# Priberam/Enhance-CB-Whisper

Hardware: AMD Instinct MI355X
Metric: utterances/sec (30 s clips) + keywords/sec matched, Whisper-large-v3 LEF 10k kw (higher is better)
Workload: dtype bf16

## Files before the change

### enhance-cb-whisper_amd/cbw/_lib.py

```python
from __future__ import annotations

import ctypes
import os

import torch

_HERE = os.path.dirname(os.path.abspath(__file__))
LIB_PATH = os.environ.get("CBW_LIB", os.path.join(_HERE, "libcbw.so"))

c_int, c_int64, c_float, c_void_p, c_char_p = ctypes.c_int, ctypes.c_int64, ctypes.c_float, ctypes.c_void_p, ctypes.c_char_p


class KwsConfig(ctypes.Structure):
    _fields_ = [("n_layers", c_int), ("embedding_dim", c_int), ("variant", c_int), ("proj_units", c_int),
                ("resnet_depth", c_int)]


class EncoderConfig(ctypes.Structure):
    _fields_ = [("n_mel", c_int), ("d_model", c_int), ("n_layers", c_int), ("n_heads", c_int), ("ffn_dim", c_int)]


class DecoderConfig(ctypes.Structure):
    _fields_ = [("vocab", c_int), ("d_model", c_int), ("n_layers", c_int), ("n_heads", c_int), ("ffn_dim", c_int),
                ("max_len", c_int)]
# ... 17 lines not shown
    "cbw_kws_rescore": (c_int, [c_void_p, c_void_p, c_void_p, c_void_p, c_void_p, c_int, c_int, c_int, c_void_p, c_int,
                                c_void_p, c_void_p, c_int64, c_void_p]),
    "cbw_kws_calibrate_bias": (c_int, [c_void_p, c_void_p, c_void_p, c_void_p, c_void_p, c_int, c_int, c_int, c_void_p,
                                       c_int, c_void_p, c_int64, c_void_p]),
    "cbw_kws_rescore_x3_workspace_bytes": (c_int64, [c_void_p, c_int, c_int]),
    "cbw_kws_rescore_x3": (c_int, [c_void_p, c_void_p, c_void_p, c_void_p, c_void_p, c_int, c_int, c_int, c_void_p,
                                   c_int, c_void_p, c_void_p, c_int64, c_void_p]),
    "cbw_kws_workspace_bytes": (c_int64, [c_void_p, c_int, c_int, c_int]),
    "cbw_kws_score": (c_int, [c_void_p, c_void_p, c_void_p, c_void_p, c_void_p, c_int, c_int, c_int, c_void_p,
                              c_void_p, c_int, c_void_p, c_int64, c_void_p]),
    "cbw_kws_classify": (c_int, [c_void_p, c_void_p, c_int, c_int, c_int, c_void_p, c_int, c_void_p, c_int64,
                                 c_void_p]),
    "cbw_kws_spot": (c_int, [c_void_p, c_void_p, c_int, c_float, c_int, c_void_p, c_void_p, c_void_p, c_void_p]),
    "cbw_checksum_workspace_bytes": (ctypes.c_int64, []),
    "cbw_checksum": (c_int, [c_void_p, ctypes.c_int64, c_void_p, c_void_p, ctypes.c_int64, c_void_p]),
    "cbw_kws_band": (c_int, [c_void_p, c_void_p, c_int, c_float, c_float, c_void_p, c_void_p, c_void_p]),
    "cbw_beam_select": (c_int, [c_void_p, c_void_p, c_int, c_int, c_int, c_void_p, c_void_p, c_void_p, c_void_p,
                                c_void_p, c_void_p, c_void_p, c_void_p, c_void_p, c_int, c_int, c_void_p]),
    "cbw_kws_set_score_offset": (c_int, [c_void_p, c_void_p]),
    "cbw_kws_band_scaled": (c_int, [c_void_p, c_void_p, c_int, c_float, c_float, c_void_p, c_void_p, c_void_p]),
    "cbw_kws_score_resized_workspace_bytes": (c_int64, [c_void_p, c_void_p, c_int, c_int, c_int, c_int, c_int, c_int]),
    "cbw_kws_score_resized": (c_int, [c_void_p, c_void_p, c_int, c_void_p, c_int, c_int, c_void_p, c_void_p, c_int,
                                      c_int, c_int, c_void_p, c_int, c_void_p, c_int64, c_void_p]),
    "cbw_mel": (c_int, [c_void_p, c_int64, c_int, c_void_p, c_void_p, c_int, c_void_p, c_void_p]),
    "cbw_mel_long": (c_int, [c_void_p, c_int64, c_int, c_void_p, c_void_p, c_void_p]),
    "cbw_encoder_create": (c_int, [ctypes.POINTER(EncoderConfig), ctypes.POINTER(c_void_p)]),
    "cbw_encoder_destroy": (c_int, [c_void_p]),
    "cbw_encoder_set_param": (c_int, [c_void_p, c_char_p, c_void_p, c_int64]),
    "cbw_encoder_finalize": (c_int, [c_void_p]),
    "cbw_encoder_workspace_bytes": (c_int64, [c_void_p, c_int]),
    "cbw_encoder_hs": (c_int, [c_void_p, c_void_p, c_int, c_void_p, c_int, c_int, c_void_p, c_void_p, c_int64,
                               c_void_p]),
    "cbw_conv2d": (c_int, [c_void_p, c_void_p, c_void_p, c_void_p, c_void_p] + [c_int] * 12 + [c_void_p]),
    "cbw_conv1x1_dual": (c_int, [c_void_p] * 6 + [c_int] * 10 + [c_void_p]),
    "cbw_gemm_splitk_factor": (c_int, [c_int, c_int, c_int]),
    "cbw_gemm": (c_int, [c_void_p] * 5 + [c_int] * 5 + [c_void_p, c_int64, c_void_p]),
    "cbw_encoder_attention": (c_int, [c_void_p, c_void_p, c_int, c_int, c_int, c_void_p]),
    "cbw_kws_profile": (c_int, [c_void_p, c_int]),
    "cbw_decoder_create": (c_int, [ctypes.POINTER(DecoderConfig), ctypes.POINTER(c_void_p)]),
    "cbw_decoder_destroy": (c_int, [c_void_p]),
    "cbw_decoder_set_param": (c_int, [c_void_p, c_char_p, c_void_p, c_int64]),
    "cbw_decoder_finalize": (c_int, [c_void_p]),
    "cbw_decoder_vocab_padded": (c_int, [c_void_p]),
    "cbw_decoder_state_bytes": (c_int64, [c_void_p, c_int, c_int]),
    "cbw_decoder_cross_kv": (c_int, [c_void_p, c_void_p, c_int, c_void_p, c_int64, c_int, c_void_p]),
    "cbw_decoder_step": (c_int, [c_void_p, c_void_p, c_int, c_int, c_int, c_void_p, c_int64, c_void_p, c_void_p]),
    "cbw_decoder_step_dev": (c_int, [c_void_p, c_void_p, c_void_p, c_int, c_int, c_void_p, c_int64, c_void_p, c_void_p]),
    "cbw_decoder_prefill": (c_int, [c_void_p, c_void_p, c_int, c_int, c_int, c_void_p, c_int64, c_void_p, c_void_p]),
    "cbw_decoder_cross_kv_slot": (c_int, [c_void_p, c_void_p, c_int, c_int, c_void_p, c_int64, c_int, c_void_p]),
    "cbw_decoder_prefill_rows": (c_int, [c_void_p, c_void_p, c_int, c_int, c_int, c_int, c_int, c_int, c_void_p, c_int64,
                                         c_void_p, c_void_p]),
    "cbw_decoder_step_rows": (c_int, [c_void_p, c_void_p, c_void_p, c_int, c_int, c_void_p, c_int64, c_void_p, c_void_p]),
    "cbw_decoder_reorder": (c_int, [c_void_p, c_void_p, c_int, c_int, c_int, c_void_p, c_int64, c_void_p]),
    "cbw_decoder_cross_attn_probs": (c_int, [c_void_p, c_void_p, c_int, c_void_p, c_int, c_int, c_int, c_void_p,
                                             c_int64, c_void_p, c_void_p]),
    "cbw_dtw": (c_int, [c_void_p, c_int, c_int, c_void_p, c_void_p, c_void_p]),
    "cbw_logprob_topk": (c_int, [c_void_p, c_int, c_int, c_int, c_void_p, c_int64, c_int, c_void_p, c_void_p, c_void_p]),
    "cbw_timestamp_rules": (c_int, [c_void_p, c_int, c_int, c_int, c_void_p, c_void_p, c_int, c_int, c_int, c_int,
                                    c_void_p, c_void_p]),
    "cbw_kws_profile_read": (c_int, [c_void_p, ctypes.POINTER(ctypes.c_double), ctypes.POINTER(ctypes.c_double), ctypes.POINTER(c_int)]),
    "cbw_kws_profile_records": (c_int, [c_void_p, c_void_p, c_void_p, c_void_p, c_int]),
    "cbw_kws_profile_tiers": (c_int, [c_void_p, c_void_p, c_int]),
    "cbw_kws_profile_kernels": (c_int, [c_void_p, c_void_p, c_int]),
    "cbw_kws_calibrate_fp8": (c_int, [c_void_p, c_void_p, c_void_p, c_void_p, c_void_p, c_int, c_int, c_int, c_void_p,
                                      c_int, c_float, c_void_p, c_int64, c_void_p]),
    "cbw_kws_score_fp8": (c_int, [c_void_p, c_void_p, c_void_p, c_void_p, c_void_p, c_int, c_int, c_int, c_void_p,
# ... 63 lines not shown
```

### enhance-cb-whisper_amd/csrc/cbw_kernels.h

```cpp
#pragma once
#include <hip/hip_runtime.h>
#include <stdint.h>

#include <initializer_list>
#include <string>

typedef __bf16 bf16;

enum {
    CBW_EPI_RELU = 1,
    CBW_EPI_GELU = 2,
    CBW_EPI_RES_F32 = 4,
    CBW_EPI_OUT_F32 = 8,
    CBW_EPI_RES_AFTER_ACT = 16,
    CBW_EPI_SPLIT3 = 32,
    CBW_EPI_RES_SPLIT = 64
};

struct ConvArgs {
    const void* x;
    const void* w;
    const float* bias;
    const void* res;
    void* y;
// ... 49 lines not shown
int cbw_gemv_waves(int K);
bool cbw_gemv_ln_ok(int M, int K);
hipError_t cbw_gemv(const GemvArgs& a, hipStream_t st);

struct F8ConvArgs {
    const uint8_t* x;
    const uint8_t* w;
    const float* alpha;
    const float* bias;
    const uint8_t* res;
    float res_scale;
    void* y;
    float y_inv_scale;
    int out_bf16;
    const void* zero;
    int N, H, W, Cin, Ho, Wo, Cout, KH, KW, sh, sw, ph, pw, M;
    int relu;
};
bool cbw_conv_fp8_supported(const F8ConvArgs& a);
bool cbw_conv_fp8_stream_supported(const F8ConvArgs& a);
hipError_t cbw_conv_fp8_stream(const F8ConvArgs& a, hipStream_t st);
hipError_t cbw_conv_fp8(const F8ConvArgs& a, hipStream_t st);
hipError_t cbw_quant_fp8(const uint16_t* x, uint8_t* y, int64_t n, float inv_scale, hipStream_t st);
int cbw_absmax_groups();
hipError_t cbw_absmax_f32(const float* x, int64_t n, float* part, hipStream_t st);
hipError_t cbw_mfma_fp8_probe(const uint8_t* A, const uint8_t* Bt, float* C, int mode, hipStream_t st);
hipError_t cbw_cvt_fp8_probe(const float* x, uint8_t* q, float* back, int n, hipStream_t st);

bool cbw_conv_ring_supported(const ConvArgs& a);
hipError_t cbw_conv_ring(const ConvArgs& a, hipStream_t st);
bool cbw_conv_stream_supported(const ConvArgs& a);
bool cbw_conv_stream_wanted(const ConvArgs& a);
hipError_t cbw_conv_stream(const ConvArgs& a, hipStream_t st);

hipError_t cbw_bottleneck_s1(const uint16_t* x, uint16_t* y, const uint16_t* wr, const float* br, const uint16_t* wm,
                             const float* bm, const uint16_t* we, const float* be, const void* zero, int N, int H,
                             int W, hipStream_t st);
hipError_t cbw_bottleneck_s1_q8(const uint16_t* x, uint8_t* y, const uint16_t* wr, const float* br, const uint16_t* wm,
                                const float* bm, const uint16_t* we, const float* be, float inv_scale, int N, int H,
                                int W, hipStream_t st);
hipError_t cbw_bottleneck_s1_first(const uint16_t* x, uint16_t* y, const uint16_t* wr, const float* br,
                                   const uint16_t* wm, const float* bm, const uint16_t* wcat, const float* bcat,
                                   const void* zero, int N, int H, int W, hipStream_t st);

hipError_t cbw_cast_permute_lbtd(const float* x, uint16_t* y, int B, int L, int T, int D, hipStream_t st);
hipError_t cbw_normalize_rows(const void* x, int x_is_f32, void* y, int y_is_f32, int L, int B, int T, int E,
                              float eps, int permute_lb, hipStream_t st);
hipError_t cbw_nchw_to_nhwc4(const float* x, uint16_t* y, int K, int L, int H, int W, hipStream_t st);
hipError_t cbw_l2norm_rows_f32(float* x, int64_t rows, int E, hipStream_t st);
hipError_t cbw_lef_time_project(const float* x, const float* w, const float* b, void* y, int y_is_f32,
                                const float* mask_in, float* mask_out,
                                int L, int B, int T, int U, float eps, hipStream_t st);
hipError_t cbw_sim_maps(const uint16_t* kwd, const float* kwd_mask, const uint16_t* utt, const float* utt_mask,
                        uint16_t* out, int K, int L, int Tk, int Tu, int E, hipStream_t st);
hipError_t cbw_sim_to_nchw(const uint16_t* maps, float* out, int K, int L, int Tk, int Tu, hipStream_t st);
hipError_t cbw_stem_conv(const uint16_t* x, const uint16_t* w, const float* bias, uint16_t* y,
                         int N, int H, int W, int Ho, int Wo, hipStream_t st);
hipError_t cbw_stem_pool(const uint16_t* x, const uint16_t* w, const float* bias, uint16_t* y, int N, int H, int W,
                         int Hs, int Ws, int Hp, int Wp, hipStream_t st);
hipError_t cbw_stem16_pool(const uint16_t* x, const uint16_t* w, const float* bias, uint16_t* y, int N, int H,
                           int W, int Hs, int Ws, int Hp, int Wp, hipStream_t st);
hipError_t cbw_stem16_pool_x3(const uint16_t* x, const uint16_t* w, const float* bias, uint16_t* y, int N, int H,
                              int W, int Hs, int Ws, int Hp, int Wp, hipStream_t st);
hipError_t cbw_maps_split16(const float* x, uint16_t* y, int K, int L, int H, int W, hipStream_t st);
hipError_t cbw_sim_resize(const float* sim, int64_t layer_stride, int ld, const int* off_dev, int k0, int K, int L,
                          int Tu, int Ho, int Wo, uint16_t* out, hipStream_t st);
// ... 68 lines not shown
```

### enhance-cb-whisper_amd/csrc/conv_stream.hip

```cpp
#include "cbw_common.h"
#include "cbw_kernels.h"

typedef int cs_i32x4 __attribute__((ext_vector_type(4)));
__device__ cs_i32x4 cs_raw_load(cs_i32x4 rsrc, int voffset, int soffset, int aux)
    __asm("llvm.amdgcn.raw.buffer.load.v4i32");
__device__ void cs_raw_store(cs_i32x4 vdata, cs_i32x4 rsrc, int voffset, int soffset, int aux)
    __asm("llvm.amdgcn.raw.buffer.store.v4i32");

namespace {

constexpr int CS_NSTEP = 64;
constexpr int CS_WBYTES = 131072;
constexpr int CS_MAXSLICE = 1024;

CBW_DEV cs_i32x4 cs_rsrc(const void* base, uint32_t bytes) {
    const uint64_t p = (uint64_t)base;
    cs_i32x4 r{(int)(uint32_t)p, (int)(uint32_t)(p >> 32), (int)bytes, 0x00020000};
#pragma unroll
    for (int q = 0; q < 4; ++q) r[q] = __builtin_amdgcn_readfirstlane(r[q]);
    return r;
}
CBW_DEV cs_i32x4 cs_load(cs_i32x4 rsrc, int voff, int soff) { return cs_raw_load(rsrc, voff, soff, 0); }
CBW_DEV void cs_store(cs_i32x4 v, cs_i32x4 rsrc, int voff, int soff) { cs_raw_store(v, rsrc, voff, soff, 0); }

// ... 116 lines not shown
            }
#pragma unroll
            for (int h = 0; h < 2; ++h) {
                const int nl = s * CS_NSTEP + h * 32 + fq * 8;
                const f32x4 bv0 = *(const f32x4*)(bias_s + nl), bv1 = *(const f32x4*)(bias_s + nl + 4);
#pragma unroll
                for (int pf = 0; pf < PF; ++pf) {
                    float v[8];
#pragma unroll
                    for (int q = 0; q < 4; ++q) {
                        v[q] = acc[pf][2 * h][q] + bv0[q];
                        v[4 + q] = acc[pf][2 * h + 1][q] + bv1[q];
                    }
                    if (has_res) {
                        const bf16x8 rv = __builtin_bit_cast(bf16x8, rs[pf][h]);
#pragma unroll
                        for (int q = 0; q < 8; ++q) v[q] += bf2f(rv[q]);
                    }
                    bf16x8 o;
#pragma unroll
                    for (int q = 0; q < 8; ++q) o[q] = f2bf(relu ? fmaxf(v[q], 0.f) : v[q]);
                    const int yo = (exp & 2) ? (v[0] == 12345.f ? yoff[pf] : OOR) : yoff[pf];
                    cs_store(__builtin_bit_cast(cs_i32x4, o), yr, yo, (n_lo + s * CS_NSTEP + h * 32) * 2);
                }
            }
            if (has_res && s + RD < nsteps) load_res(rs, s + RD);
        };
        for (int s = 0; s < nsteps; s += RD) {
            if (PN && s + RD >= nsteps && u + ustride < units) load_rows(u + ustride, xn, roffn, yoffn);
#pragma unroll
            for (int r = 0; r < RD; ++r) step(res[r], s + r);
        }
    }
}

int num_cus_cs() {
    static int n = 0;
    if (n == 0) {
        int dev = 0;
        (void)hipGetDevice(&dev);
        if (hipDeviceGetAttribute(&n, hipDeviceAttributeMultiprocessorCount, dev) != hipSuccess || n <= 0) n = 256;
        const char* e = getenv("CBW_CS_CUS");
        if (e && atoi(e) > 0) n = std::min(n, atoi(e));
    }
    return n;
}

int cs_exp() {
    const char* e = getenv("CBW_CS_EXP");
    return e ? atoi(e) : 0;
}

int stream_prefetch() {
    const char* e = getenv("CBW_CS_PREFETCH");
    return e ? atoi(e) : -1;
}

int stream_k512() {
    const char* e = getenv("CBW_CS_K512");
    return e ? atoi(e) : 1;
}

int stream_mode() {
    const char* e = getenv("CBW_CONV_STREAM");
    return e ? atoi(e) : 1;
}
// ... 35 lines not shown
    const int ktot = a.Cin + (a.x2 ? a.Cin2 : 0);
    const int sn = slice_channels(a.Cout, ktot);
    const int nslice = a.Cout / sn;
    const int cus = cbw_cs_grid_cus > 0 ? std::min(num_cus_cs(), cbw_cs_grid_cus) : num_cus_cs();
    const int G = 8 * nslice * std::max(1, cus / (8 * nslice));
    const size_t lds = (size_t)sn * ktot * 2 + (size_t)sn * 4;
    const int pf = stream_prefetch();
    const int pn = pf >= 0 ? pf : (ktot == 128 || (ktot == 256 && !a.res));
#define CS_LAUNCH(KS, WAVES, RD, PFD, PN)                                                                               \
    do {                                                                                                           \
        cbw_last_conv_kernel = "conv_stream_kernel<" #KS ", " #WAVES ", " #RD ", " #PFD ", " #PN ">";                \
        hipLaunchKernelGGL((conv_stream_kernel<KS, WAVES, RD, PFD, PN>), dim3(G), dim3(WAVES * 64), lds, st, a,       \
                           nslice, sn, cs_exp());                                                                  \
    } while (0)
    switch (ktot) {
        case 128:
            if (pn) CS_LAUNCH(4, 8, 2, 2, 1);
            else CS_LAUNCH(4, 12, 2, 2, 0);
            break;
        case 256:
            if (pn) CS_LAUNCH(8, 8, 1, 2, 1);
            else CS_LAUNCH(8, 12, 1, 2, 0);
            break;
        case 512:
            CS_LAUNCH(16, 8, 2, 1, 0);
            break;
        default:
            CS_LAUNCH(12, 8, 2, 2, 0);
            break;
    }
#undef CS_LAUNCH
    return hipGetLastError();
}
```

### enhance-cb-whisper_amd/csrc/runtime.cpp

```cpp
#include <hip/hip_runtime.h>

#include <algorithm>
#include <cmath>
#include <cstring>
#include <limits>
#include <map>
#include <memory>
#include <string>
#include <vector>

#include "cbw.h"
#include "cbw_kernels.h"

namespace {

thread_local std::string g_err;

int fail(int code, const std::string& msg) {
    g_err = msg;
    return code;
}

#define HIPCHK(expr)                                                                                   \
    do {                                                                                               \
// ... 153 lines not shown
    int cin, H, W, stride;
};

int launch_conv(const ConvW& c, const void* x, int N, int H, int W, void* y, const void* res, int flags,
                const void* zero, hipStream_t st, int* Ho_out = nullptr, int* Wo_out = nullptr, Prof* prof = nullptr,
                const Src2* src2 = nullptr, float* splitk_ws = nullptr) {
    ConvArgs a{};
    a.x = x; a.w = c.w.p; a.bias = c.b.as<float>(); a.res = res; a.y = y; a.zero = zero;
    if (src2) { a.x2 = src2->x; a.Cin2 = src2->cin; a.H2 = src2->H; a.W2 = src2->W; a.s2 = src2->stride; }
    a.N = N; a.H = H; a.W = W; a.Cin = c.cin; a.Cout = c.cout; a.KH = c.k; a.KW = c.k;
    a.sh = a.sw = c.stride; a.ph = a.pw = c.k / 2;
    a.Ho = (H + 2 * a.ph - a.KH) / a.sh + 1;
    a.Wo = (W + 2 * a.pw - a.KW) / a.sw + 1;
    a.M = N * a.Ho * a.Wo;
    a.res_ld = a.y_ld = c.cout;
    a.flags = flags | (c.relu ? CBW_EPI_RELU : 0);
    if (Ho_out) *Ho_out = a.Ho;
    if (Wo_out) *Wo_out = a.Wo;
    const bool rec = prof && prof->on && (size_t)(2 * prof->used + 1) < prof->ev.size();
    if (rec) HIPCHK(hipEventRecord(prof->ev[2 * prof->used], st));
    cbw_last_conv_kernel = "?";
    if (splitk_ws) HIPCHK(cbw_conv_igemm_splitk(a, cbw_conv_splitk_factor(a), splitk_ws, st));
    else HIPCHK(cbw_conv_igemm(a, st));
    if (rec) {
        HIPCHK(hipEventRecord(prof->ev[2 * prof->used + 1], st));
        prof->flop[prof->used] = 2.0 * a.M * a.Cout * ((double)a.Cin * a.KH * a.KW + (a.x2 ? a.Cin2 : 0));
        prof->tier[prof->used] = prof->cur_tier;
        prof->kern[prof->used] = cbw_last_conv_kernel;
        prof->used++;
    }
    return CBW_OK;
}

size_t align_up(size_t n) { return (n + 255) & ~(size_t)255; }

struct BlockW {
    ConvW conv[3];
    int nconv = 0;
    bool has_sc = false;
    bool fused_sc = false;
    ConvW sc;
    std::string prefix;
    int stage = 0;
};

struct ConvF8 {
    DevBuf w, alpha, b;
    int cin = 0, cout = 0, k = 1, stride = 1;
    bool relu = false;
};
struct BlockF8 {
    ConvF8 conv[3];
    bool has_sc = false;
    ConvF8 sc;
    float s_x = 1.f, s_t1 = 1.f, s_t2 = 1.f, s_sc = 1.f;
    float s_out = 1.f;
    bool out_bf16 = false;
};

struct ConvW32 {
    DevBuf w, b;
    int cin = 0, cout = 0, k = 1, stride = 1;
    bool relu = false;
};
struct BlockW32 {
    ConvW32 conv[3];
    int nconv = 0;
    bool has_sc = false;
    ConvW32 sc;
};

int load_conv_bn32(const ParamStore& ps, const std::string& prefix, ConvW32& c) {
    std::vector<float> o, sh;
    CHK(fold_conv_host(ps, prefix, c.cin, c.cout, c.k, o, sh));
// ... 194 lines not shown
                        o[((co * 7 + kh) * 8 + kw) * C + c] = (*w)[((co * L + c) * 7 + kh) * 7 + kw] * sc[co];
        CHK(h->stem_w.upload(to_bf16(o)));
        CHK(h->stem_b.upload(sh));
    }
    h->blocks.clear();
    int cin = 64;
    for (size_t s = 0; s < hs.size(); ++s) {
        const int cout = hs[s];
        for (int li = 0; li < depths[s]; ++li) {
            const int stride = (li == 0 && s > 0) ? 2 : 1;
            const std::string p = root + ".encoder.stages." + std::to_string(s) + ".layers." + std::to_string(li);
            BlockW b;
            b.prefix = p;
            b.stage = (int)s + 1;
            if (cin != cout || stride != 1) {
                b.has_sc = true;
                b.sc.cin = cin; b.sc.cout = cout; b.sc.k = 1; b.sc.stride = stride; b.sc.relu = false;
                CHK(load_conv_bn(h->ps, p + ".shortcut", b.sc));
            }
            if (bottleneck) {
                const int mid = cout / 4;
                const int ci[3] = {cin, mid, mid}, co[3] = {mid, mid, cout}, k[3] = {1, 3, 1}, st[3] = {1, stride, 1};
                const bool rl[3] = {true, true, false};
                b.nconv = 3;
                for (int j = 0; j < 3; ++j) {
                    b.conv[j].cin = ci[j]; b.conv[j].cout = co[j]; b.conv[j].k = k[j]; b.conv[j].stride = st[j];
                    b.conv[j].relu = rl[j];
                    if (j == 2 && b.has_sc && cout % 128 == 0 && sc_fusion_enabled()) {
                        CHK(load_fused_expand_shortcut(h->ps, p + ".layer.2", p + ".shortcut", mid, cin, cout, b.conv[2]));
                        b.fused_sc = true;
                    } else {
                        CHK(load_conv_bn(h->ps, p + ".layer." + std::to_string(j), b.conv[j]));
                    }
                }
            } else {
                b.nconv = 2;
                b.conv[0].cin = cin; b.conv[0].cout = cout; b.conv[0].k = 3; b.conv[0].stride = stride; b.conv[0].relu = true;
                b.conv[1].cin = cout; b.conv[1].cout = cout; b.conv[1].k = 3; b.conv[1].stride = 1; b.conv[1].relu = false;
                for (int j = 0; j < 2; ++j) CHK(load_conv_bn(h->ps, p + ".layer." + std::to_string(j), b.conv[j]));
            }
            h->blocks.push_back(std::move(b));
            cin = cout;
        }
    }
    int rc;
    const auto* fw = h->ps.get("model.classifier.1.weight", (size_t)2 * h->hidden, &rc);
    if (!fw) return rc;
    const auto* fb = h->ps.get("model.classifier.1.bias", 2, &rc);
    if (!fb) return rc;
    CHK(h->fc_w.upload(*fw));
    CHK(h->fc_b.upload(*fb));
    CHK(h->fc_b16.upload(*fb));
    CHK(h->fc_b8.upload(*fb));
    return CBW_OK;
}

int build_projector(cbw_kws* h) {
    const int L = h->cfg.n_layers, D = h->cfg.embedding_dim, U = h->cfg.proj_units;
    h->p1.clear();
    h->p2.clear();
    h->p1.resize(L);
    h->p2.resize(L);
    for (int l = 0; l < L; ++l) {
        int rc;
        const std::string p = "projector." + std::to_string(l);
        const auto* w1 = h->ps.get(p + ".0.weight", (size_t)(D / 2) * D, &rc); if (!w1) return rc;
// ... 318 lines not shown
                        nullptr, 0, h->zero.p, st));
        CHK(launch_conv(h->p2[l], h1 + (size_t)l * rows_l * (D / 2), 1, 1, (int)rows_l, h2 + (size_t)l * rows_l * U,
                        nullptr, CBW_EPI_OUT_F32, h->zero.p, st));
    }
    if (h->cfg.variant == 1) {
        HIPCHK(cbw_normalize_rows(h2, 1, out, 0, L, B, T, U, eps, 1, st));
        HIPCHK(hipMemcpyAsync(mask_out, mask, sizeof(float) * B * L * T, hipMemcpyDeviceToDevice, st));
    } else {
        HIPCHK(cbw_lef_time_project(h2, h->tp_w.as<float>(), h->tp_b.as<float>(), out, 0, mask, mask_out, L, B, T, U, eps,
                                    st));
    }
    return CBW_OK;
}

}

namespace {
int64_t chunk_ws_bytes(const cbw_kws* h, int Tk, int Tu, int chunk) {
    const KwsPlan p = kws_plan(h, Tk, Tu, chunk);
    return (int64_t)(align_up(p.maps * 2) + 3 * align_up(p.big * 2) + 2 * align_up(p.small * 2));
}
}

extern "C" {

int64_t cbw_kws_workspace_bytes(cbw_kws* h, int Tk, int Tu, int chunk) {
    if (!h || !h->finalized || chunk <= 0) return -1;
    return kws_streams() * chunk_ws_bytes(h, Tk, Tu, chunk);
}

namespace {
int cs_shared_cus() {
    const char* e = getenv("CBW_CS_SHARED_CUS");
    return e ? atoi(e) : 96;
}
struct ChunkStreams {
    cbw_kws* h;
    hipStream_t st;
    int n;
    int saved_cus;
    static int balanced(int want, int nchunks) {
        const int n = std::max(1, std::min(want, nchunks));
        const int rounds = (nchunks + n - 1) / n;
        return std::max(1, (nchunks + rounds - 1) / rounds);
    }
    ChunkStreams(cbw_kws* h_, hipStream_t st_, int nchunks)
        : h(h_), st(st_), n(h_->fork_ev ? balanced(kws_streams(), nchunks) : 1), saved_cus(cbw_cs_grid_cus) {
        if (n > 1) cbw_cs_grid_cus = cs_shared_cus();
    }
    ~ChunkStreams() { cbw_cs_grid_cus = saved_cus; }
    ChunkStreams(const ChunkStreams&) = delete;
    ChunkStreams& operator=(const ChunkStreams&) = delete;
    int begin() {
        if (n > 1) {
            HIPCHK(hipEventRecord(h->fork_ev, st));
            for (int i = 0; i + 1 < n; ++i) {
                if (!h->side[i]) HIPCHK(side_stream_create(&h->side[i]));
                HIPCHK(hipStreamWaitEvent(h->side[i], h->fork_ev, 0));
            }
        }
        return CBW_OK;
    }
    hipStream_t stream(int i) const { return (i % n) ? h->side[i % n - 1] : st; }
    int slot(int i) const { return i % n; }
    int end() {
        for (int i = 0; i + 1 < n; ++i) {
            HIPCHK(hipEventRecord(h->join_ev[i], h->side[i]));
// ... 5 lines not shown

int resnet_chunk(cbw_kws* h, const KwsPlan& plan, char* ws, int kc, int Tk, int Tu, float* logits, hipStream_t st,
                 bool fp8 = false) {
    char* p = ws + align_up(plan.maps * 2);
    uint16_t* maps = (uint16_t*)ws;
    uint16_t* X = (uint16_t*)p; p += align_up(plan.big * 2);
    uint16_t* Y = (uint16_t*)p; p += align_up(plan.big * 2);
    uint16_t* SC = (uint16_t*)p; p += align_up(plan.big * 2);
    uint16_t* T1 = (uint16_t*)p; p += align_up(plan.small * 2);
    uint16_t* T2 = (uint16_t*)p;
    const int Hs = (Tk + 6 - 7) / 2 + 1, Ws = (Tu + 6 - 7) / 2 + 1;
    const int Hp = (Hs - 1) / 2 + 1, Wp = (Ws - 1) / 2 + 1;
    const int L = h->cfg.n_layers;

    auto stem = [&](int n0, int nn) -> int {
        uint16_t* xo = X + (size_t)n0 * Hp * Wp * 64;
        const uint16_t* mo = maps + (size_t)n0 * Tk * Tu * stem_channels(L);
        if (stem_channels(L) == 16) {
            HIPCHK(cbw_stem16_pool(mo, h->stem_w.as<uint16_t>(), h->stem_b.as<float>(), xo, nn, Tk, Tu, Hs, Ws, Hp, Wp,
                                   st));
        } else if (stem_fusion_enabled()) {
            HIPCHK(cbw_stem_pool(mo, h->stem_w.as<uint16_t>(), h->stem_b.as<float>(), xo, nn, Tk, Tu, Hs, Ws, Hp, Wp,
                                 st));
        } else {
            uint16_t* yo = Y + (size_t)n0 * Hs * Ws * 64;
            HIPCHK(cbw_stem_conv(mo, h->stem_w.as<uint16_t>(), h->stem_b.as<float>(), yo, nn, Tk, Tu, Hs, Ws, st));
            HIPCHK(cbw_maxpool3s2(yo, xo, nn, Hs, Ws, 64, Hp, Wp, st));
        }
        return CBW_OK;
    };
    auto blocks = [&](size_t b0, size_t b1, int n0, int nn, uint16_t*& x, uint16_t*& y, int& H, int& W,
                      int& C) -> int {
        auto at = [&](uint16_t* base, int hh, int ww, int cc) { return base + (size_t)n0 * hh * ww * cc; };
        for (size_t bi = b0; bi < b1; ++bi) {
            const auto& b = h->blocks[bi];
            uint16_t* xo = at(x, H, W, C);
            int Ho = H, Wo = W;
            const void* res = xo;
            const bool s1_first = b.nconv == 3 && b.has_sc && b.fused_sc && b.sc.stride == 1 && b.sc.cin == 64 &&
                                  b.conv[0].cin == 64 && b.conv[0].cout == 64 && b.conv[1].stride == 1 &&
                                  b.conv[2].cout == 256 && bottleneck_fusion_enabled() && bottleneck_first_enabled();
            if (b.has_sc && !b.fused_sc) {
                const int hs = (H - 1) / b.sc.stride + 1, ws2 = (W - 1) / b.sc.stride + 1;
                uint16_t* sco = at(SC, hs, ws2, b.sc.cout);
                CHK(launch_conv(b.sc, xo, nn, H, W, sco, nullptr, 0, h->zero.p, st, nullptr, nullptr, &h->prof));
                res = sco;
            }
            if (s1_first || (b.nconv == 3 && !b.has_sc && b.conv[0].cin == 256 && b.conv[0].cout == 64 &&
                             b.conv[2].cout == 256 && bottleneck_fusion_enabled())) {
                uint16_t* yo = at(y, H, W, 256);
                const bool rec = h->prof.on && (size_t)(2 * h->prof.used + 1) < h->prof.ev.size();
                if (rec) HIPCHK(hipEventRecord(h->prof.ev[2 * h->prof.used], st));
                if (s1_first)
                    HIPCHK(cbw_bottleneck_s1_first(xo, yo, b.conv[0].w.as<uint16_t>(), b.conv[0].b.as<float>(),
                                                   b.conv[1].w.as<uint16_t>(), b.conv[1].b.as<float>(),
                                                   b.conv[2].w.as<uint16_t>(), b.conv[2].b.as<float>(), h->zero.p, nn,
                                                   H, W, st));
                else
                    HIPCHK(cbw_bottleneck_s1(xo, yo, b.conv[0].w.as<uint16_t>(), b.conv[0].b.as<float>(),
                                             b.conv[1].w.as<uint16_t>(), b.conv[1].b.as<float>(),
                                             b.conv[2].w.as<uint16_t>(), b.conv[2].b.as<float>(), h->zero.p, nn, H, W,
                                             st));
                if (rec) {
                    HIPCHK(hipEventRecord(h->prof.ev[2 * h->prof.used + 1], st));
                    const double cin = s1_first ? 64.0 : 256.0;
                    h->prof.flop[h->prof.used] =
                        2.0 * nn * H * W * (cin * 64 + 64.0 * 576 + 64.0 * 256 + (s1_first ? 64.0 * 256 : 0.0));
                    h->prof.tier[h->prof.used] = h->prof.cur_tier;
                    h->prof.kern[h->prof.used] = s1_first ? "bottleneck_kernel<64>" : "bottleneck_ring_kernel";
                    h->prof.used++;
                }
            } else if (b.nconv == 3) {
                const auto &c0 = b.conv[0], &c1 = b.conv[1], &c2 = b.conv[2];
                const int h1 = (H + 2 * (c0.k / 2) - c0.k) / c0.stride + 1, w1 = (W + 2 * (c0.k / 2) - c0.k) / c0.stride + 1;
                Ho = (h1 + 2 * (c1.k / 2) - c1.k) / c1.stride + 1;
                Wo = (w1 + 2 * (c1.k / 2) - c1.k) / c1.stride + 1;
                uint16_t* t1 = at(T1, h1, w1, c0.cout);
                uint16_t* t2 = at(T2, Ho, Wo, c1.cout);
                uint16_t* yo = at(y, Ho, Wo, c2.cout);
                CHK(launch_conv(c0, xo, nn, H, W, t1, nullptr, 0, h->zero.p, st, nullptr, nullptr, &h->prof));
                CHK(launch_conv(c1, t1, nn, h1, w1, t2, nullptr, 0, h->zero.p, st, nullptr, nullptr, &h->prof));
                if (b.fused_sc) {
                    const Src2 s2{xo, b.sc.cin, H, W, b.sc.stride};
                    CHK(launch_conv(c2, t2, nn, Ho, Wo, yo, nullptr, CBW_EPI_RELU, h->zero.p, st, nullptr, nullptr,
                                    &h->prof, &s2));
                } else {
                    CHK(launch_conv(c2, t2, nn, Ho, Wo, yo, res, CBW_EPI_RELU, h->zero.p, st, nullptr, nullptr,
                                    &h->prof));
                }
            } else {
                const auto &c0 = b.conv[0], &c1 = b.conv[1];
                Ho = (H + 2 * (c0.k / 2) - c0.k) / c0.stride + 1;
                Wo = (W + 2 * (c0.k / 2) - c0.k) / c0.stride + 1;
                uint16_t* t1 = at(T1, Ho, Wo, c0.cout);
                uint16_t* yo = at(y, Ho, Wo, c1.cout);
                CHK(launch_conv(c0, xo, nn, H, W, t1, nullptr, 0, h->zero.p, st, nullptr, nullptr, &h->prof));
                CHK(launch_conv(c1, t1, nn, Ho, Wo, yo, res, CBW_EPI_RELU, h->zero.p, st, nullptr, nullptr, &h->prof));
            }
            std::swap(x, y);
            H = Ho;
            W = Wo;
            C = b.conv[b.nconv - 1].cout;
        }
        return CBW_OK;
    };

    if (fp8) {
        int H = Hp, W = Wp, C = 64;
        uint16_t *x = X, *y = Y;
        CHK(stem(0, kc));
        if (h->f8_first < 1) return fail(CBW_ERR_STATE, "fp8 tier: no bf16 stage before the e4m3 blocks");
        const size_t lb = (size_t)h->f8_first - 1;
        const auto& b1 = h->blocks[lb];
        const bool q8 = fp8_q8_enabled() && b1.nconv == 3 && !b1.has_sc && b1.conv[0].cin == 256 &&
                        b1.conv[0].cout == 64 && b1.conv[2].cout == 256 && bottleneck_fusion_enabled();
// ... 1675 lines not shown
    HIPCHK(hipGetDevice(&dev));
    auto it = zeros.find(dev);
    if (it == zeros.end()) {
        auto z = std::make_shared<DevBuf>();
        CHK(z->alloc(256));
        HIPCHK(hipMemset(z->p, 0, 256));
        it = zeros.emplace(dev, z).first;
    }
    *out = it->second->p;
    return CBW_OK;
}
}
extern "C" {
int cbw_conv2d(const uint16_t* x, const uint16_t* w, const float* bias, const void* res, void* y, int N, int H, int W,
               int Cin, int Cout, int KH, int KW, int sh, int sw, int ph, int pw, int flags, cbw_stream_t stream) {
    if (!x || !w || !y || Cin % 64 || Cout % 64) return fail(CBW_ERR_INVALID, "cbw_conv2d: Cin and Cout must be multiples of 64");
    if (!((KH == 1 && KW == 1) || (KH == 3 && KW == 3) || (KH == 1 && KW == 3)))
        return fail(CBW_ERR_INVALID, "cbw_conv2d: kernel must be 1x1, 3x3 or 1x3");
    const void* zp = nullptr;
    CHK(block_zero_page(&zp));
    ConvArgs a{};
    a.x = x; a.w = w; a.bias = bias; a.res = res; a.y = y; a.zero = zp;
    a.N = N; a.H = H; a.W = W; a.Cin = Cin; a.Cout = Cout; a.KH = KH; a.KW = KW;
    a.sh = sh; a.sw = sw; a.ph = ph; a.pw = pw;
    a.Ho = (H + 2 * ph - KH) / sh + 1;
    a.Wo = (W + 2 * pw - KW) / sw + 1;
    a.M = N * a.Ho * a.Wo;
    a.res_ld = a.y_ld = Cout;
    a.flags = flags;
    HIPCHK(cbw_conv_igemm(a, (hipStream_t)stream));
    return CBW_OK;
}

int cbw_gemm_splitk_factor(int M, int K, int N) {
    if (M <= 0 || K <= 0 || N <= 0) return fail(CBW_ERR_INVALID, "cbw_gemm_splitk_factor: bad shape");
    ConvArgs a{};
    a.KH = a.KW = 1; a.Cin = K; a.Cout = N; a.M = M;
    return cbw_conv_splitk_factor(a);
}

int cbw_encoder_attention(const uint16_t* qkv, uint16_t* out, int B, int T, int H, cbw_stream_t stream) {
    if (!qkv || !out || B <= 0 || T <= 0 || H <= 0) return fail(CBW_ERR_INVALID, "cbw_encoder_attention: bad argument");
    HIPCHK(cbw_attention(qkv, out, B, T, H, 64, (hipStream_t)stream));
    return CBW_OK;
}

int cbw_gemm(const uint16_t* x, const uint16_t* w, const float* bias, const void* res, void* y, int M, int K, int N,
             int flags, int ksplit, float* partial, int64_t partial_floats, cbw_stream_t stream) {
    if (!x || !w || !y || M <= 0 || K % 64 || N % 64 || ksplit < 0)
        return fail(CBW_ERR_INVALID, "cbw_gemm: K and N must be multiples of 64");
    const void* zp = nullptr;
    CHK(block_zero_page(&zp));
    ConvArgs a{};
    a.x = x; a.w = w; a.bias = bias; a.res = res; a.y = y; a.zero = zp;
    a.N = 1; a.H = 1; a.W = M; a.Cin = K; a.Cout = N; a.KH = a.KW = 1;
    a.sh = a.sw = 1; a.ph = a.pw = 0; a.Ho = 1; a.Wo = M; a.M = M;
    a.res_ld = a.y_ld = N;
    a.flags = flags;
    const int S = ksplit == 0 ? cbw_conv_splitk_factor(a) : ksplit;
    if (S > 1) {
        if (!partial || partial_floats < (int64_t)S * M * N) return fail(CBW_ERR_OOM, "cbw_gemm: partial buffer too small");
        if (N % 128 || S > K / 64) return fail(CBW_ERR_INVALID, "cbw_gemm: split-K needs N % 128 == 0 and S <= K / 64");
    }
    HIPCHK(cbw_conv_igemm_splitk(a, S, partial, (hipStream_t)stream));
    return CBW_OK;
}
// ... 24 lines not shown
```

### include/cbw.h

```cpp
#ifndef CBW_H
#define CBW_H
#include <stdint.h>

#ifdef __cplusplus
extern "C" {
#endif

#define CBW_OK 0
#define CBW_ERR_INVALID (-1)
#define CBW_ERR_HIP (-2)
#define CBW_ERR_OOM (-3)
#define CBW_ERR_STATE (-4)
#define CBW_ERR_NOT_FOUND (-5)

typedef void* cbw_stream_t;
typedef struct cbw_kws cbw_kws;
typedef struct cbw_encoder cbw_encoder;

int cbw_version(void);
const char* cbw_last_error(void);
const char* cbw_source_id(void);

typedef struct {
    int n_layers;
// ... 95 lines not shown
int64_t cbw_decoder_state_bytes(cbw_decoder* h, int B, int Benc);
int cbw_decoder_cross_kv(cbw_decoder* h, const float* enc_out, int Benc, void* state, int64_t state_bytes, int B,
                         cbw_stream_t stream);
int cbw_decoder_step(cbw_decoder* h, const int32_t* tokens, int pos, int B, int Benc, void* state, int64_t state_bytes,
                     float* logits, cbw_stream_t stream);
int cbw_decoder_step_dev(cbw_decoder* h, const int32_t* tokens, const int32_t* pos_dev, int B, int Benc, void* state,
                         int64_t state_bytes, float* logits, cbw_stream_t stream);
int cbw_decoder_prefill(cbw_decoder* h, const int32_t* tokens, int T, int B, int Benc, void* state,
                        int64_t state_bytes, float* logits, cbw_stream_t stream);
int cbw_decoder_cross_kv_slot(cbw_decoder* h, const float* enc_out, int slot, int Benc, void* state,
                              int64_t state_bytes, int B, cbw_stream_t stream);
int cbw_decoder_prefill_rows(cbw_decoder* h, const int32_t* tokens, int T, int slot, int r0, int nb, int B, int Benc,
                             void* state, int64_t state_bytes, float* logits, cbw_stream_t stream);
int cbw_decoder_step_rows(cbw_decoder* h, const int32_t* tokens, const int32_t* pos_rows, int B, int Benc, void* state,
                          int64_t state_bytes, float* logits, cbw_stream_t stream);
int cbw_decoder_cross_attn_probs(cbw_decoder* h, const int32_t* tokens, int T, const int32_t* heads, int n, int B,
                                 int Benc, void* state, int64_t state_bytes, float* probs, cbw_stream_t stream);
int cbw_dtw(const double* matrix, int rows, int cols, int32_t* text_idx, int32_t* time_idx, int* len);
int cbw_decoder_reorder(cbw_decoder* h, const int32_t* src_rows, int B, int Benc, int len, void* state,
                        int64_t state_bytes, cbw_stream_t stream);
int cbw_logprob_topk(const float* logits, int B, int V, int ld, const float* bias, int64_t bias_ld, int k, float* lp,
                     int32_t* idx, cbw_stream_t stream);
int cbw_timestamp_rules(const float* logits, int B, int V, int ld, const float* bias, const int32_t* state,
                        int timestamp_begin, int no_timestamps, int eos, int max_initial, float* bias_out,
                        cbw_stream_t stream);

int cbw_beam_select(const float* lp, const int32_t* idx, int B, int k, int eos, double* beam_scores,
                    double* cand_score, int32_t* cand_row, int32_t* cand_tok, int32_t* tokens, int32_t* parents,
                    int32_t* ok, int32_t* ts_state, int32_t* st_out, int timestamp_begin, int count,
                    cbw_stream_t stream);

int cbw_conv2d(const uint16_t* x, const uint16_t* w, const float* bias, const void* res, void* y, int N, int H, int W,
               int Cin, int Cout, int KH, int KW, int sh, int sw, int ph, int pw, int flags, cbw_stream_t stream);
int cbw_conv2d_fp8(const uint8_t* x, const uint8_t* w, const float* alpha, const float* bias, const uint8_t* res,
                   float res_scale, void* y, float y_scale, int out_bf16, int relu, int N, int H, int W, int Cin,
                   int Cout, int k, int stride, cbw_stream_t stream);
int cbw_fp8_probe(int what, const void* a, const void* b, void* out, void* out2, int n, cbw_stream_t stream);

int cbw_conv1x1_dual(const uint16_t* x, const uint16_t* x2, const uint16_t* w, const float* bias, const void* res,
                     void* y, int N, int H, int W, int Cin, int H2, int W2, int Cin2, int s2, int Cout, int flags,
                     cbw_stream_t stream);
int cbw_gemm_splitk_factor(int M, int K, int N);
int cbw_gemm(const uint16_t* x, const uint16_t* w, const float* bias, const void* res, void* y, int M, int K, int N,
             int flags, int ksplit, float* partial, int64_t partial_floats, cbw_stream_t stream);
int cbw_encoder_attention(const uint16_t* qkv, uint16_t* out, int B, int T, int H, cbw_stream_t stream);

#ifdef __cplusplus
}
#endif
#endif
```

Before: 6.130.

## Fuse bottleneck expand conv with next block's reduce conv in one streaming kernel

Adds a chained 1x1 conv kernel that computes a bottleneck block's 128→512 expand conv (bias, residual add, ReLU) and feeds each output tile straight into the next block's 512→128 reduce conv via MFMA, writing both outputs. This avoids re-reading the 512-channel activation and one kernel launch per consecutive identity-block pair. The reduce weights are pre-packed into MFMA fragment order at load time. It also changes the default shared-CU count for chunk streams from a fixed value to 3/8 of the device CU count. The fused kernel keeps a large per-wave register working set, which limits occupancy.

```diff
diff --git a/enhance-cb-whisper_amd/cbw/_lib.py b/enhance-cb-whisper_amd/cbw/_lib.py
--- a/enhance-cb-whisper_amd/cbw/_lib.py
+++ b/enhance-cb-whisper_amd/cbw/_lib.py
@@ -73,6 +73,7 @@
     "cbw_encoder_hs": (c_int, [c_void_p, c_void_p, c_int, c_void_p, c_int, c_int, c_void_p, c_void_p, c_int64,
                                c_void_p]),
     "cbw_conv2d": (c_int, [c_void_p, c_void_p, c_void_p, c_void_p, c_void_p] + [c_int] * 12 + [c_void_p]),
+    "cbw_conv1x1_chain": (c_int, [c_void_p] * 8 + [c_int] * 3 + [c_void_p]),
     "cbw_conv1x1_dual": (c_int, [c_void_p] * 6 + [c_int] * 10 + [c_void_p]),
     "cbw_gemm_splitk_factor": (c_int, [c_int, c_int, c_int]),
     "cbw_gemm": (c_int, [c_void_p] * 5 + [c_int] * 5 + [c_void_p, c_int64, c_void_p]),
diff --git a/enhance-cb-whisper_amd/csrc/cbw_kernels.h b/enhance-cb-whisper_amd/csrc/cbw_kernels.h
--- a/enhance-cb-whisper_amd/csrc/cbw_kernels.h
+++ b/enhance-cb-whisper_amd/csrc/cbw_kernels.h
@@ -105,6 +105,10 @@
 bool cbw_conv_stream_supported(const ConvArgs& a);
 bool cbw_conv_stream_wanted(const ConvArgs& a);
 hipError_t cbw_conv_stream(const ConvArgs& a, hipStream_t st);
+bool cbw_conv_chain_enabled();
+bool cbw_conv_chain_supported(const ConvArgs& a, int red_cout);
+hipError_t cbw_conv_chain_pack(const uint16_t* wr, uint16_t* packed, hipStream_t st);
+hipError_t cbw_conv_chain(const ConvArgs& a, const uint16_t* wr_packed, const float* br, void* t1, hipStream_t st);
 
 hipError_t cbw_bottleneck_s1(const uint16_t* x, uint16_t* y, const uint16_t* wr, const float* br, const uint16_t* wm,
                              const float* bm, const uint16_t* we, const float* be, const void* zero, int N, int H,
diff --git a/enhance-cb-whisper_amd/csrc/conv_stream.hip b/enhance-cb-whisper_amd/csrc/conv_stream.hip
--- a/enhance-cb-whisper_amd/csrc/conv_stream.hip
+++ b/enhance-cb-whisper_amd/csrc/conv_stream.hip
@@ -172,6 +172,152 @@
             for (int r = 0; r < RD; ++r) step(res[r], s + r);
         }
     }
+}
+
+constexpr int CC_K = 128, CC_N = 512, CC_R = 128;
+template <int WAVES, int RD, int PF>
+__global__ __launch_bounds__(WAVES * 64, 1) void conv_stream_chain_kernel(ConvArgs a, const bf16* __restrict__ wrp,
+                                                                          const float* __restrict__ br, void* t1) {
+    extern __shared__ __attribute__((aligned(16))) char smem[];
+    constexpr int KS = CC_K / 32;
+    constexpr int PITCH = CC_K * 2;
+    constexpr int NSTEPS = CC_N / CS_NSTEP;
+    constexpr int RF = CC_R / 16;
+    float* bias_s = (float*)(smem + CC_N * PITCH);
+    float* br_s = bias_s + CC_N;
+    const int tid = threadIdx.x, lane = tid & 63, wid = tid >> 6;
+    const int fr = lane & 15, fq = lane >> 4;
+
+    const bf16* __restrict__ Wt = (const bf16*)a.w;
+    constexpr int CPR = CC_K / 8;
+    for (int e = tid; e < CC_N * CPR; e += WAVES * 64) {
+        const int r = e / CPR, c = e - r * CPR;
+        *(bf16x8*)(smem + cs_off(r, c, PITCH)) = *(const bf16x8*)(Wt + (int64_t)perm_row(r) * CC_K + c * 8);
+    }
+    for (int c = tid; c < CC_N; c += WAVES * 64) bias_s[c] = a.bias ? a.bias[c] : 0.f;
+    for (int c = tid; c < CC_R; c += WAVES * 64) br_s[c] = br ? br[c] : 0.f;
+    __syncthreads();
+
+    const int M = a.M;
+    const int units = (M + (PF * 16) - 1) / (PF * 16);
+    const cs_i32x4 xr = cs_rsrc(a.x, (uint32_t)((int64_t)M * CC_K * 2));
+    const cs_i32x4 rr = cs_rsrc(a.res, (uint32_t)((int64_t)M * a.res_ld * 2));
+    const cs_i32x4 yr = cs_rsrc(a.y, (uint32_t)((int64_t)M * a.y_ld * 2));
+    const cs_i32x4 tr = cs_rsrc(t1, (uint32_t)((int64_t)M * CC_R * 2));
+    const cs_i32x4 wr = cs_rsrc(wrp, (uint32_t)(CC_R * CC_N * 2));
+    constexpr int OOR = 0x7ffffff0;
+
+    const int ustride = gridDim.x * WAVES;
+    for (int u = blockIdx.x * WAVES + wid; u < units; u += ustride) {
+        int roff[PF], yoff[PF], toff[PF];
+        bf16x8 xf[PF][KS];
+#pragma unroll
+        for (int pf = 0; pf < PF; ++pf) {
+            const int p = u * (PF * 16) + pf * 16 + fr;
+            const bool ok = p < M;
+            const int xo = ok ? p * CC_K * 2 + fq * 16 : OOR;
+            roff[pf] = ok ? p * a.res_ld * 2 + fq * 16 : OOR;
+            yoff[pf] = ok ? p * a.y_ld * 2 + fq * 16 : OOR;
+            toff[pf] = ok ? p * CC_R * 2 + fq * 16 : OOR;
+#pragma unroll
+            for (int ks = 0; ks < KS; ++ks) xf[pf][ks] = __builtin_bit_cast(bf16x8, cs_load(xr, xo, ks * 64));
+        }
+        cs_i32x4 res[RD][PF][2];
+        auto load_res = [&](cs_i32x4 (&dst)[PF][2], int s) {
+#pragma unroll
+            for (int pf = 0; pf < PF; ++pf)
+#pragma unroll
+                for (int h = 0; h < 2; ++h) dst[pf][h] = cs_load(rr, roff[pf], (s * CS_NSTEP + h * 32) * 2);
+        };
+#pragma unroll
+        for (int r = 0; r < RD; ++r) load_res(res[r], r);
+        auto load_wr = [&](cs_i32x4 (&dst)[RF], int kk) {
+#pragma unroll
+            for (int c = 0; c < RF; ++c) dst[c] = cs_load(wr, lane * 16, (kk * RF + c) * 1024);
+        };
+        f32x4 tacc[PF][RF];
+#pragma unroll
+        for (int pf = 0; pf < PF; ++pf)
+#pragma unroll
+            for (int c = 0; c < RF; ++c) tacc[pf][c] = f32x4{0.f, 0.f, 0.f, 0.f};
+        auto step = [&](cs_i32x4 (&rs)[PF][2], int s) {
+            cs_i32x4 wr0[RF], wr1[RF];
+            load_wr(wr0, 2 * s);
+            f32x4 acc[PF][4];
+#pragma unroll
+            for (int pf = 0; pf < PF; ++pf)
+#pragma unroll
+                for (int c = 0; c < 4; ++c) acc[pf][c] = f32x4{0.f, 0.f, 0.f, 0.f};
+#pragma unroll
+            for (int ks = 0; ks < KS; ++ks) {
+                bf16x8 wf[4];
+#pragma unroll
+                for (int c = 0; c < 4; ++c)
+                    wf[c] = *(const bf16x8*)(smem + cs_off(s * CS_NSTEP + c * 16 + fr, ks * 4 + fq, PITCH));
+#pragma unroll
+                for (int c = 0; c < 4; ++c)
+#pragma unroll
+                    for (int pf = 0; pf < PF; ++pf)
+                        acc[pf][c] = __builtin_amdgcn_mfma_f32_16x16x32_bf16(wf[c], xf[pf][ks], acc[pf][c], 0, 0, 0);
+            }
+            load_wr(wr1, 2 * s + 1);
+#pragma unroll
+            for (int h = 0; h < 2; ++h) {
+                const int nl = s * CS_NSTEP + h * 32 + fq * 8;
+                const f32x4 bv0 = *(const f32x4*)(bias_s + nl), bv1 = *(const f32x4*)(bias_s + nl + 4);
+#pragma unroll
+                for (int pf = 0; pf < PF; ++pf) {
+                    float v[8];
+#pragma unroll
+                    for (int q = 0; q < 4; ++q) {
+                        v[q] = acc[pf][2 * h][q] + bv0[q];
+                        v[4 + q] = acc[pf][2 * h + 1][q] + bv1[q];
+                    }
+                    const bf16x8 rv = __builtin_bit_cast(bf16x8, rs[pf][h]);
+#pragma unroll
+                    for (int q = 0; q < 8; ++q) v[q] += bf2f(rv[q]);
+                    bf16x8 o;
+#pragma unroll
+                    for (int q = 0; q < 8; ++q) o[q] = f2bf(fmaxf(v[q], 0.f));
+                    cs_store(__builtin_bit_cast(cs_i32x4, o), yr, yoff[pf], (s * CS_NSTEP + h * 32) * 2);
+#pragma unroll
+                    for (int c = 0; c < RF; ++c)
+                        tacc[pf][c] = __builtin_amdgcn_mfma_f32_16x16x32_bf16(
+                            __builtin_bit_cast(bf16x8, h ? wr1[c] : wr0[c]), o, tacc[pf][c], 0, 0, 0);
+                }
+            }
+            if (s + RD < NSTEPS) load_res(rs, s + RD);
+        };
+        for (int s = 0; s < NSTEPS; s += RD) {
+#pragma unroll
+            for (int r = 0; r < RD; ++r) step(res[r], s + r);
+        }
+#pragma unroll
+        for (int t = 0; t < CC_R / 64; ++t)
+#pragma unroll
+            for (int h = 0; h < 2; ++h) {
+                const int nl = t * 64 + h * 32 + fq * 8;
+                const f32x4 bv0 = *(const f32x4*)(br_s + nl), bv1 = *(const f32x4*)(br_s + nl + 4);
+#pragma unroll
+                for (int pf = 0; pf < PF; ++pf) {
+                    bf16x8 o;
+#pragma unroll
+                    for (int q = 0; q < 4; ++q) {
+                        o[q] = f2bf(fmaxf(tacc[pf][4 * t + 2 * h][q] + bv0[q], 0.f));
+                        o[4 + q] = f2bf(fmaxf(tacc[pf][4 * t + 2 * h + 1][q] + bv1[q], 0.f));
+                    }
+                    cs_store(__builtin_bit_cast(cs_i32x4, o), tr, toff[pf], (t * 64 + h * 32) * 2);
+                }
+            }
+    }
+}
+
+__global__ void conv_chain_pack_kernel(const bf16* __restrict__ w, bf16* __restrict__ out) {
+    const int e = blockIdx.x * blockDim.x + threadIdx.x;
+    if (e >= CC_R * CC_N / 8) return;
+    const int lane = e & 63, c = (e >> 6) & 7, kk = e >> 9;
+    const int fr = lane & 15, fq = lane >> 4;
+    *(bf16x8*)(out + (int64_t)e * 8) = *(const bf16x8*)(w + (int64_t)perm_row(16 * c + fr) * CC_N + kk * 32 + fq * 8);
 }
 
 int num_cus_cs() {
@@ -273,3 +419,31 @@
 #undef CS_LAUNCH
     return hipGetLastError();
 }
+
+bool cbw_conv_chain_enabled() {
+    const char* e = getenv("CBW_CS_CHAIN");
+    return !e || atoi(e) != 0;
+}
+
+bool cbw_conv_chain_supported(const ConvArgs& a, int red_cout) {
+    if (!cbw_conv_stream_supported(a) || a.x2 || a.Cin != CC_K || a.Cout != CC_N || red_cout != CC_R) return false;
+    if (!a.res || a.flags != CBW_EPI_RELU || a.y_ld != CC_N) return false;
+    return slice_channels(a.Cout, a.Cin) == a.Cout;
+}
+
+hipError_t cbw_conv_chain_pack(const uint16_t* wr, uint16_t* packed, hipStream_t st) {
+    hipLaunchKernelGGL(conv_chain_pack_kernel, dim3(CC_R * CC_N / 8 / 256), dim3(256), 0, st, (const bf16*)wr,
+                       (bf16*)packed);
+    return hipGetLastError();
+}
+
+hipError_t cbw_conv_chain(const ConvArgs& a, const uint16_t* wr_packed, const float* br, void* t1, hipStream_t st) {
+    if (!cbw_conv_chain_supported(a, CC_R) || !wr_packed || !t1) return hipErrorNotSupported;
+    const int cus = cbw_cs_grid_cus > 0 ? std::min(num_cus_cs(), cbw_cs_grid_cus) : num_cus_cs();
+    const int G = 8 * std::max(1, cus / 8);
+    const size_t lds = (size_t)CC_N * CC_K * 2 + (size_t)(CC_N + CC_R) * 4;
+    cbw_last_conv_kernel = "conv_stream_chain_kernel<4, 2, 4>";
+    hipLaunchKernelGGL((conv_stream_chain_kernel<4, 2, 4>), dim3(G), dim3(4 * 64), lds, st, a, (const bf16*)wr_packed, br,
+                       t1);
+    return hipGetLastError();
+}
diff --git a/enhance-cb-whisper_amd/csrc/runtime.cpp b/enhance-cb-whisper_amd/csrc/runtime.cpp
--- a/enhance-cb-whisper_amd/csrc/runtime.cpp
+++ b/enhance-cb-whisper_amd/csrc/runtime.cpp
@@ -209,6 +209,38 @@
     return CBW_OK;
 }
 
+int launch_chain(const ConvW& c2, const ConvW& r0, const DevBuf& r0_packed, const void* t2, int N, int H, int W, void* y,
+                 const void* res, void* t1n, const void* zero, hipStream_t st, Prof* prof, bool* done) {
+    *done = false;
+    if (!r0_packed.p || !res || !cbw_conv_chain_enabled()) return CBW_OK;
+    if (c2.k != 1 || c2.stride != 1 || c2.relu || r0.k != 1 || r0.stride != 1 || !r0.relu || r0.cin != c2.cout)
+        return CBW_OK;
+    ConvArgs a{};
+    a.x = t2; a.w = c2.w.p; a.bias = c2.b.as<float>(); a.res = res; a.y = y; a.zero = zero;
+    a.N = N; a.H = a.Ho = H; a.W = a.Wo = W; a.Cin = c2.cin; a.Cout = c2.cout; a.KH = a.KW = 1;
+    a.sh = a.sw = 1;
+    a.M = N * H * W;
+    a.res_ld = a.y_ld = c2.cout;
+    a.flags = CBW_EPI_RELU;
+    ConvArgs r = a;
+    r.x = y; r.w = r0.w.p; r.bias = r0.b.as<float>(); r.res = nullptr; r.y = t1n;
+    r.Cin = r0.cin; r.Cout = r0.cout; r.res_ld = r.y_ld = r0.cout;
+    if (!cbw_conv_stream_wanted(a) || !cbw_conv_stream_wanted(r) || !cbw_conv_chain_supported(a, r0.cout)) return CBW_OK;
+    const bool rec = prof && prof->on && (size_t)(2 * prof->used + 1) < prof->ev.size();
+    if (rec) HIPCHK(hipEventRecord(prof->ev[2 * prof->used], st));
+    cbw_last_conv_kernel = "?";
+    HIPCHK(cbw_conv_chain(a, r0_packed.as<uint16_t>(), r0.b.as<float>(), t1n, st));
+    if (rec) {
+        HIPCHK(hipEventRecord(prof->ev[2 * prof->used + 1], st));
+        prof->flop[prof->used] = 2.0 * a.M * a.Cout * (double)a.Cin + 2.0 * a.M * r0.cout * (double)r0.cin;
+        prof->tier[prof->used] = prof->cur_tier;
+        prof->kern[prof->used] = cbw_last_conv_kernel;
+        prof->used++;
+    }
+    *done = true;
+    return CBW_OK;
+}
+
 size_t align_up(size_t n) { return (n + 255) & ~(size_t)255; }
 
 struct BlockW {
@@ -217,6 +249,7 @@
     bool has_sc = false;
     bool fused_sc = false;
     ConvW sc;
+    DevBuf chain_w;
     std::string prefix;
     int stage = 0;
 };
@@ -477,6 +510,11 @@
                     } else {
                         CHK(load_conv_bn(h->ps, p + ".layer." + std::to_string(j), b.conv[j]));
                     }
+                }
+                if (!b.has_sc && cin == 512 && mid == 128) {
+                    CHK(b.chain_w.alloc((size_t)mid * cin * 2));
+                    HIPCHK(cbw_conv_chain_pack(b.conv[0].w.as<uint16_t>(), b.chain_w.as<uint16_t>(), nullptr));
+                    HIPCHK(hipStreamSynchronize(nullptr));
                 }
             } else {
                 b.nconv = 2;
@@ -861,7 +899,11 @@
 namespace {
 int cs_shared_cus() {
     const char* e = getenv("CBW_CS_SHARED_CUS");
-    return e ? atoi(e) : 96;
+    if (e) return atoi(e);
+    int dev = 0, n = 0;
+    (void)hipGetDevice(&dev);
+    if (hipDeviceGetAttribute(&n, hipDeviceAttributeMultiprocessorCount, dev) != hipSuccess || n <= 0) n = 256;
+    return n * 3 / 8;
 }
 struct ChunkStreams {
     cbw_kws* h;
@@ -933,6 +975,7 @@
     auto blocks = [&](size_t b0, size_t b1, int n0, int nn, uint16_t*& x, uint16_t*& y, int& H, int& W,
                       int& C) -> int {
         auto at = [&](uint16_t* base, int hh, int ww, int cc) { return base + (size_t)n0 * hh * ww * cc; };
+        bool t1_ready = false;
         for (size_t bi = b0; bi < b1; ++bi) {
             const auto& b = h->blocks[bi];
             uint16_t* xo = at(x, H, W, C);
@@ -979,9 +1022,16 @@
                 uint16_t* t1 = at(T1, h1, w1, c0.cout);
                 uint16_t* t2 = at(T2, Ho, Wo, c1.cout);
                 uint16_t* yo = at(y, Ho, Wo, c2.cout);
-                CHK(launch_conv(c0, xo, nn, H, W, t1, nullptr, 0, h->zero.p, st, nullptr, nullptr, &h->prof));
+                if (!t1_ready) CHK(launch_conv(c0, xo, nn, H, W, t1, nullptr, 0, h->zero.p, st, nullptr, nullptr, &h->prof));
                 CHK(launch_conv(c1, t1, nn, h1, w1, t2, nullptr, 0, h->zero.p, st, nullptr, nullptr, &h->prof));
-                if (b.fused_sc) {
+                t1_ready = false;
+                if (!b.has_sc && bi + 1 < b1 && h->blocks[bi + 1].nconv == 3 && !h->blocks[bi + 1].has_sc) {
+                    const auto& nb = h->blocks[bi + 1];
+                    CHK(launch_chain(c2, nb.conv[0], nb.chain_w, t2, nn, Ho, Wo, yo, res, at(T1, Ho, Wo, nb.conv[0].cout),
+                                     h->zero.p, st, &h->prof, &t1_ready));
+                }
+                if (t1_ready) {
+                } else if (b.fused_sc) {
                     const Src2 s2{xo, b.sc.cin, H, W, b.sc.stride};
                     CHK(launch_conv(c2, t2, nn, Ho, Wo, yo, nullptr, CBW_EPI_RELU, h->zero.p, st, nullptr, nullptr,
                                     &h->prof, &s2));
@@ -2723,6 +2773,28 @@
     return CBW_OK;
 }
 
+int cbw_conv1x1_chain(const uint16_t* x, const uint16_t* we, const float* be, const uint16_t* res, const uint16_t* wr,
+                      const float* br, uint16_t* y, uint16_t* t1, int N, int H, int W, cbw_stream_t stream) {
+    if (!x || !we || !be || !res || !wr || !br || !y || !t1 || N <= 0 || H <= 0 || W <= 0)
+        return fail(CBW_ERR_INVALID, "cbw_conv1x1_chain: bad argument");
+    const void* zp = nullptr;
+    CHK(block_zero_page(&zp));
+    ConvArgs a{};
+    a.x = x; a.w = we; a.bias = be; a.res = res; a.y = y; a.zero = zp;
+    a.N = N; a.H = a.Ho = H; a.W = a.Wo = W; a.Cin = 128; a.Cout = 512; a.KH = a.KW = 1;
+    a.sh = a.sw = 1;
+    a.M = N * H * W;
+    a.res_ld = a.y_ld = 512;
+    a.flags = CBW_EPI_RELU;
+    if (!cbw_conv_chain_supported(a, 128)) return fail(CBW_ERR_INVALID, "cbw_conv1x1_chain: shape not supported");
+    DevBuf packed;
+    CHK(packed.alloc((size_t)128 * 512 * 2));
+    HIPCHK(cbw_conv_chain_pack(wr, packed.as<uint16_t>(), (hipStream_t)stream));
+    HIPCHK(cbw_conv_chain(a, packed.as<uint16_t>(), br, t1, (hipStream_t)stream));
+    HIPCHK(hipStreamSynchronize((hipStream_t)stream));
+    return CBW_OK;
+}
+
 int cbw_gemm_splitk_factor(int M, int K, int N) {
     if (M <= 0 || K <= 0 || N <= 0) return fail(CBW_ERR_INVALID, "cbw_gemm_splitk_factor: bad shape");
     ConvArgs a{};
diff --git a/include/cbw.h b/include/cbw.h
--- a/include/cbw.h
+++ b/include/cbw.h
@@ -151,6 +151,8 @@
 
 int cbw_conv2d(const uint16_t* x, const uint16_t* w, const float* bias, const void* res, void* y, int N, int H, int W,
                int Cin, int Cout, int KH, int KW, int sh, int sw, int ph, int pw, int flags, cbw_stream_t stream);
+int cbw_conv1x1_chain(const uint16_t* x, const uint16_t* we, const float* be, const uint16_t* res, const uint16_t* wr,
+                      const float* br, uint16_t* y, uint16_t* t1, int N, int H, int W, cbw_stream_t stream);
 int cbw_conv2d_fp8(const uint8_t* x, const uint8_t* w, const float* alpha, const float* bias, const uint8_t* res,
                    float res_scale, void* y, float y_scale, int out_bf16, int relu, int N, int H, int W, int Cin,
                    int Cout, int k, int stride, cbw_stream_t stream);
```

After: 6.193, median of 6. 1.0% higher.
